# epsilla-cloud/vectordb

Measured on AMD Instinct MI355X. Metric: QPS @ recall@10>=0.999, 10Mx768 L2, higher is better.
Workload: dtype f32 (exact fp32 distances; the batched scan runs an int8 MFMA pass (int32 accumulation) over an 8-bit mirror of the rows as a lower-bound filter, survivors re-ranked in fp32)

## Files before the change

### vectordb_amd/build.py

```python
import os
import subprocess
import sys
from concurrent.futures import ThreadPoolExecutor

HERE = os.path.dirname(os.path.abspath(__file__))
SRC = os.path.join(HERE, "csrc")
OUT = os.path.join(HERE, "lib")
OBJ = os.path.join(OUT, "obj")
LIB = os.path.join(OUT, "libepsilla_gfx950.so")
SOURCES = ["index.cpp", "index_calls.cpp", "c_abi.cpp", "shard_group.cpp", "exchange.cpp", "flat_kernels.hip", "traverse.hip", "mfma_filter.hip", "one_pass.hip",
           "mirror_build.hip", "graph_build.hip", "select.hip", "range.hip"]
FLAGS = ["--offload-arch=gfx950", "-O3", "-std=c++17", "-fPIC", "-fno-gpu-rdc", "-Wall", "-Wno-unused-function",
         "-I" + os.path.join(os.path.dirname(HERE), "include")]


def _hipcc():
    for c in (os.environ.get("HIPCC"), "/opt/rocm/bin/hipcc", "hipcc"):
        if c and (os.path.sep not in c or os.path.exists(c)):
            return c
    raise RuntimeError("hipcc not found")


def _stale(target, deps):
    if not os.path.exists(target):
        return True
    t = os.path.getmtime(target)
    return any(os.path.getmtime(d) > t for d in deps)


def build(force=False, verbose=False):
    os.makedirs(OBJ, exist_ok=True)
    hipcc = _hipcc()
    headers = [os.path.join(SRC, f) for f in os.listdir(SRC) if f.endswith((".hpp", ".h"))]
    headers.append(os.path.join(os.path.dirname(HERE), "include", "epsilla_gfx950.h"))
    jobs = []
    objs = []
    for s in SOURCES:
        src = os.path.join(SRC, s)
        obj = os.path.join(OBJ, s.rsplit(".", 1)[0] + ".o")
        objs.append(obj)
        if force or _stale(obj, [src] + headers):
            cmd = [hipcc] + FLAGS + (["-x", "hip"] if s.endswith(".cpp") else []) + ["-c", src, "-o", obj]
            jobs.append(cmd)
# ... 21 lines not shown
```

### vectordb_amd/csrc/flat_kernels.hip

```cpp
#include "kernels.hpp"
#include "stream8_kernel.hpp"

namespace eps {

template <int NQ, int KPL>
__device__ __forceinline__ void offer(WaveTopK<KPL> (&list)[NQ], u64 (&thr)[NQ], int q, u64 key, bool valid,
                                      const FilterSpec& f, int k, bool unique) {
  u64 m = __ballot(valid && key < thr[q]);
  while (m) {
    const int l = __ffsll((long long)m) - 1;
    m &= m - 1;
    const u64 x = shfl64(key, l);
    if (x < thr[q] && row_visible(f, key_id(x), key_dist(x))) {
      if (unique) list[q].insert_unique(x); else list[q].insert(x);
      const u64 kth = list[q].entry(k - 1);
      thr[q] = kth < thr[q] ? kth : thr[q];
    }
  }
}

template <int NQ, int KPL, bool VEC4, int U>
__global__ __launch_bounds__(256) void flat_scan_kernel(FlatScanArgs a) {
  extern __shared__ __attribute__((aligned(16))) float smem[];
  const int dim = a.dim;
// ... 72 lines not shown
  if (gx_cap < 1) gx_cap = 1;
  int64_t gx = gx_rows < gx_cap ? gx_rows : gx_cap;
  return (int)(gx * 4);
}

template <int NQ, int KPL>
static void launch_flat_scan_t(const FlatScanArgs& a, bool vec4, hipStream_t s) {
  const int gx = a.W / 4;
  const int64_t groups = (a.nq + NQ - 1) / NQ;
  dim3 grid(gx, (unsigned)groups);
  const size_t shm = (size_t)NQ * ((a.dim + 3) & ~3) * sizeof(float);
  if (vec4)
    hipLaunchKernelGGL((flat_scan_kernel<NQ, KPL, true, 4>), grid, dim3(256), shm, s, a);
  else
    hipLaunchKernelGGL((flat_scan_kernel<NQ, KPL, false, 4>), grid, dim3(256), shm, s, a);
}

void launch_flat_scan(const FlatScanArgs& a, hipStream_t s) {
  if (a.nq <= 0 || a.row_end <= a.row_begin) return;
  const bool vec4 = (a.dim % 4 == 0) && ((reinterpret_cast<uintptr_t>(a.rows) & 15) == 0);
  const int kpl = pick_kpl(a.k);
  const int nq = pick_nq(a.nq, a.k, a.dim);
#define EPS_CASE(NQ_, KPL_) \
  if (nq == NQ_ && kpl == KPL_) return launch_flat_scan_t<NQ_, KPL_>(a, vec4, s);
  EPS_CASE(1, 1) EPS_CASE(2, 1) EPS_CASE(4, 1)
  EPS_CASE(1, 2) EPS_CASE(2, 2) EPS_CASE(4, 2)
  EPS_CASE(1, 4) EPS_CASE(1, 8) EPS_CASE(1, 16)
#undef EPS_CASE
}

template <int KPL, int NW>
__global__ __launch_bounds__(NW * 64) void merge_lists_kernel(const u64* partial, int lists, int k, u64* run_keys,
                                                          int merge_run, const u32* counts, FilterSpec vis, u64 id_stride, u32 id_head,
                                                          u32* seed_cand, int seed_cap, u32* seed_cnt) {
  __shared__ u64 sh[NW][KPL * 64];
  constexpr int NT = NW * 64;
  const int64_t q = blockIdx.x;
  const int lane = lane_id();
  const int wave = threadIdx.x >> 6;
  const u64* src = partial + q * (int64_t)lists;
  int total = lists;
  if (counts) total = counts[q] < (u32)total ? (int)counts[q] : total;
  WaveTopK<KPL> L[1];
  u64 thr[1];
  L[0].init();
  thr[0] = KEY_EMPTY;
  FilterSpec nof = {nullptr, nullptr, 0, 0, 0, 0};
  if (merge_run) {
    thr[0] = run_keys[q * k + (k - 1)];
    if (wave == 0) L[0].load(run_keys + q * k, k);
  }
  const int rounded = (total + NT - 1) / NT * NT;
  for (int i = threadIdx.x; i < rounded; i += NT) {
    const u64 key = i < total ? src[i] : KEY_EMPTY;
    if (id_stride) {
      const bool ok = key != KEY_EMPTY && row_visible(vis, seed_row(key_id(key), id_head, id_stride), key_dist(key));
      offer<1, KPL>(L, thr, 0, key, ok, nof, k, false);
    } else {
      offer<1, KPL>(L, thr, 0, key, key != KEY_EMPTY, vis, k, false);
    }
  }
  L[0].store(&sh[wave][0], k);
  __syncthreads();
  if (wave == 0) {
    for (int w = 1; w < NW; ++w) {
      for (int e0 = 0; e0 < k; e0 += 64) {
        const int e = e0 + lane;
        const u64 key = e < k ? sh[w][e] : KEY_EMPTY;
        offer<1, KPL>(L, thr, 0, key, key != KEY_EMPTY, nof, k, false);
      }
    }
    if (seed_cand) {
      int c = 0;
#pragma unroll
      for (int r = 0; r < KPL; ++r) {
        const int e = r * 64 + lane;
        const u64 key = L[0].key[r];
        const bool ok = e < k && key != KEY_EMPTY;
        const unsigned long long m = __ballot(ok);
        if (ok) seed_cand[q * (int64_t)seed_cap + c + __popcll(m & ((1ull << lane) - 1ull))] = id_stride ? seed_row(key_id(key), id_head, id_stride) : key_id(key);
        c += __popcll(m);
        if (e < k) run_keys[q * k + e] = KEY_EMPTY;
      }
      if (lane == 0) seed_cnt[q] = (u32)c;
    } else {
      L[0].store(run_keys + q * k, k);
    }
  }
}

void launch_merge_lists(const u64* partial, int lists, int k, int64_t nq, u64* run_keys, bool merge_run, hipStream_t s,
                        const u32* counts, const FilterSpec* visible, u64 id_stride, u32 id_head, u32* seed_cand, int seed_cap, u32* seed_cnt) {
  const FilterSpec vis = visible ? *visible : no_filter();
  if (nq <= 0) return;
  const int kpl = pick_kpl(k);
  const bool wide = nq <= 64 && kpl <= 2;
#define EPS_CASE(KPL_) \
  if (kpl == KPL_) {   \
    if (wide && KPL_ <= 2)                                                                                                                                       \
      hipLaunchKernelGGL((merge_lists_kernel<(KPL_ <= 2 ? KPL_ : 1), 16>), dim3((unsigned)nq), dim3(1024), 0, s, partial, lists, k, run_keys, merge_run ? 1 : 0, counts, vis, \
                         id_stride, id_head, seed_cand, seed_cap, seed_cnt);                                                                                      \
    else                                                                                                                                                         \
      hipLaunchKernelGGL((merge_lists_kernel<KPL_, 4>), dim3((unsigned)nq), dim3(256), 0, s, partial, lists, k, run_keys, merge_run ? 1 : 0, counts, vis, id_stride, id_head, \
                         seed_cand, seed_cap, seed_cnt);                                                                                                          \
    return;            \
  }
  EPS_CASE(1) EPS_CASE(2) EPS_CASE(4) EPS_CASE(8) EPS_CASE(16)
#undef EPS_CASE
}

template <int KPL, bool VEC4, int NW>
__global__ __launch_bounds__(NW * 64) void rerank_kernel(RerankArgs a) {
  extern __shared__ __attribute__((aligned(16))) float smem[];
  constexpr int NT = NW * 64;
  const int dim = a.dim;
  const int qstride = (dim + 3) & ~3;
  u64* sh = reinterpret_cast<u64*>(smem + qstride);
  const int64_t q = blockIdx.x;
  for (int i = threadIdx.x; i < qstride; i += NT) smem[i] = i < dim ? a.queries[q * dim + i] : 0.f;
  if (a.fuse && a.gsync && q == 0)
    for (int i = threadIdx.x; i < 256; i += NT) a.gsync[i] = 0;
  __syncthreads();
  const int lane = lane_id();
  const int wave = threadIdx.x >> 6;
  const int G = group_lanes(dim, VEC4);
  const int RPW = 64 / G;
  const int g = lane / G;
  const int t = lane & (G - 1);
  constexpr int U = 4;
  __shared__ u32 s8_kept, s8_lost;
  __shared__ int s8_T;
  if (a.s8_G) {
    if (threadIdx.x == 0) s8_kept = s8_lost = 0;
    if (wave == 0) {
      int gk;
      const int T = stream8_threshold_of(a.s8_G + q * (a.s8_slots * S8_SLOT_STRIDE), a.k, a.qstat + q * 4, a.scal, a.metric, a.u, a.slack, lane, gk, a.s8_slots);
      if (lane == 0) s8_T = T;
// ... 382 lines not shown
```

### vectordb_amd/csrc/kernels.hpp

```cpp
#pragma once
#include <hip/hip_runtime.h>
#include <stdint.h>

#include "device_common.hpp"

namespace eps {

struct FlatScanArgs {
  const float* rows;
  int64_t row_begin, row_end;
  int dim;
  int metric;
  const float* queries;
  int64_t nq;
  int k;
  FilterSpec f;
  u64* partial;
  int W;
  const u64* thr_in;
  const u64* lo_in;
  int64_t lo_stride;
};
int flat_scan_waves(int64_t nrows, int64_t nq, int dim);
void launch_flat_scan(const FlatScanArgs& a, hipStream_t s);

void launch_merge_lists(const u64* keys, int slots, int k, int64_t nq, u64* run_keys, bool merge_run, hipStream_t s,
                        const u32* counts = nullptr, const FilterSpec* visible = nullptr, u64 id_stride = 0, u32 id_head = 0,
                        u32* seed_cand = nullptr, int seed_cap = 0, u32* seed_cnt = nullptr);

struct RerankArgs {
  const float* rows;
  int dim;
  int metric;
  const float* queries;
  int64_t nq;
  int k;
  FilterSpec f;
  const u32* cand;
  u32* cand_count;
  int cap;
  u64* run_keys;
  int fuse;
  u32* overflow;
  unsigned long long* total;
  void* T_next;
  const float* qstat;
  const float* scal;
  int bits;
  float u, slack;
  u32* gsync;
  int64_t* fin_ids = nullptr;
  float* fin_dist = nullptr;
  int32_t* fin_counts = nullptr;
  int64_t fin_base = 0, fin_stride = 1;
  const int* s8_G = nullptr;
  int s8_slots = 64;
  const u32* s8_counts = nullptr;
  const u64* s8_lists = nullptr;
  int s8_waves = 0;
  u32* s8_cand = nullptr;
  u32* pub = nullptr;
// ... 82 lines not shown
```

### vectordb_amd/csrc/mfma_filter.hip

```cpp
#include <algorithm>
#include <cmath>
#include <cstdio>
#include <cstring>
#include <numeric>
#include <vector>

#include "mirror.hpp"
#include "mfma_kernels.hpp"

namespace eps {

__global__ __launch_bounds__(256) void query_prep_kernel(const float* q, int64_t nq, int64_t b_pad, int dim, int d_pad,
                                                         _Float16* qh, float* qstat) {
  const int64_t r = (int64_t)blockIdx.x * 4 + (threadIdx.x >> 6);
  if (r >= b_pad) return;
  const int lane = lane_id();
  _Float16* dst = qh + r * d_pad;
  if (r >= nq) {
    for (int c = lane; c < d_pad; c += 64) dst[c] = (_Float16)0.f;
    if (lane == 0) qstat[r * 4 + 0] = qstat[r * 4 + 1] = qstat[r * 4 + 2] = qstat[r * 4 + 3] = 0.f;
    return;
  }
  const float* src = q + r * dim;
  float s2 = 0.f, e2 = 0.f;
// ... 114 lines not shown
    bounds.push_back(approx ? S0 : 0);
    int nstages = i8 ? (nq <= 4 ? 3 : (nq <= 64 ? 4 : 6)) : 3;
    if (i8)
      while (nstages < 8 && (double)k * 5.0 * std::pow((double)n / (double)S0, 1.0 / (double)nstages) > 0.5 * (double)cap) ++nstages;
    const double r = std::max(i8 ? 3.0 : 4.0, std::pow((double)n / (double)S0, 1.0 / (double)nstages));
    const int64_t qt = std::max<int64_t>(1, b_pad / 256);
    const int64_t unit = 256 * std::max<int64_t>(1, 256 / std::gcd<int64_t>(256, qt));
    double f = 1.0;
    for (int st = 1; st < nstages; ++st) {
      f *= r;
      int64_t bnd = (int64_t)((double)S0 * f) / ROWPAD * ROWPAD;
      if (bnd >= 2 * unit) bnd = bnd / unit * unit;
      if (bnd < n && bnd > bounds.back()) bounds.push_back(bnd);
    }
  } else {
    bounds.push_back(std::min(S0, n));
    for (int64_t bnd : {S0 * 32, S0 * 256}) {
      if (bnd < n && bnd > bounds.back()) bounds.push_back(bnd);
    }
  }
  if (bounds.back() < n) bounds.push_back(n);
  return bounds;
}

struct Chain {
  const float* dq; int64_t nq; int k; u64* run_keys;
  bool i8;
  bool approx;
  int64_t n;
  bool fold;
  bool seeded;
  bool prologue;
  bool gsync;
  int version;
  int64_t b_pad, S0;
  int cap;
  int d_pad_h;
  float u8, slack;
  CallCounters c;
  FilterSpec fs;
  std::vector<int64_t> bounds;
  bool prep_does_it_all() const { return i8 && version >= 7; }
  const float* maxima(const HalfMirror& m) const { return i8 ? (fold ? m.scal8f.as<float>() : m.scal8.as<float>()) : m.scal.as<float>(); }
  u32* group_counters(const HalfMirror& m) const { return gsync ? m.gsync.as<u32>() : nullptr; }
};

static int32_t plan_chain(Index& ix, HalfMirror& m, const float* dq, int64_t nq, int k, u64* run_keys, bool approx, int cap_scale, bool i8, int64_t n, Chain* out) {
  Chain& c = *out = Chain{dq, nq, k, run_keys, i8, approx, n};
  c.b_pad = (nq + BN3 - 1) / BN3 * BN3;
  c.cap = std::max(4096, 64 * k) * cap_scale;
  c.d_pad_h = i8 ? m.d_pad8 / 2 : m.d_pad;
  c.u8 = key_unit8(ix.metric_, m.step8);
  c.slack = rerank_slack(ix.dim_);
  const int64_t b_pad = c.b_pad;
  if (!m.qstat.reserve((size_t)b_pad * 16) || !m.T.reserve((size_t)b_pad * 4) || !m.cand.reserve((size_t)nq * c.cap * 8) ||
      !m.cnt.reserve((size_t)(nq + 4) * 4 + 16) || !m.seedc.reserve((size_t)nq * k * 4) || !(i8 ? m.q8.reserve((size_t)b_pad * m.d_pad8) : m.qh.reserve((size_t)b_pad * m.d_pad * 2)))
    return ix.fail(EPS_INFRA_UNEXPECTED_ERROR, "MFMA engine: out of device memory (scratch)");
  c.version = (c.d_pad_h % 128 != 0 || c.d_pad_h < 256) ? 3 : 7;
  if (c.version >= 7 && !m.qf.reserve((size_t)b_pad * c.d_pad_h * 2)) return ix.fail(EPS_INFRA_UNEXPECTED_ERROR, "MFMA engine: out of device memory (scratch)");
  if (!m.gsync.reserve(1024)) return ix.fail(EPS_INFRA_UNEXPECTED_ERROR, "MFMA engine: out of device memory (scratch)");
  c.S0 = seed_rows(k);
  c.seeded = !(tune_int("EPS_MFMA_SEED", 1) == 0) && n > 4 * c.S0;
  c.prologue = c.seeded && c.version >= 7;
  c.gsync = !(tune_int("EPS_MFMA_GROUPSYNC", 1) == 0);
  c.fold = i8 && !approx && m.fold8;
  c.c = call_counters(m.cnt.as<u32>(), nq);
  c.fs = ix.filter_spec();
  c.bounds = plan_stages(n, nq, k, b_pad, c.cap, i8, approx, c.seeded);
  return EPS_OK;
}

static int32_t prepare_queries(Index& ix, HalfMirror& m, const Chain& c) {
  hipStream_t s = ix.stream_;
  if (c.i8) {
    Prep8Extra px;
    if (c.prep_does_it_all()) {
      px.qf = m.qf.as<signed char>();
      if (c.prologue) {
        px.T2 = reinterpret_cast<u64*>(m.T.p);
        px.n2 = c.b_pad / 2;
        px.Tv = 0x7F8000007F800000ull;
        px.cnt = c.c.cnt;
        px.cntv = (u32)c.S0;
        px.gsync = c.group_counters(m);
      }
    }
    const hipError_t er = prep8_queries(m, c.fold, (int)ix.dim_, ix.metric_, c.dq, c.nq, c.b_pad, m.q8.as<signed char>(), m.qstat.as<float>(), px, s);
    if (er != hipSuccess) return ix.hip_fail(er, "memset");
    if (c.fold) ix.stats_.i8_folded = 1;
    ix.stats_.i8_rotated = m.rot8 ? 1 : 0;
  } else {
    hipLaunchKernelGGL(query_prep_kernel, dim3((unsigned)((c.b_pad + 3) / 4)), dim3(256), 0, s, c.dq, c.nq, c.b_pad, (int)ix.dim_,
                       m.d_pad, m.qh.as<_Float16>(), m.qstat.as<float>());
  }
  if (c.version >= 7 && !c.prep_does_it_all())
    hipLaunchKernelGGL(pack_qf_kernel, dim3((unsigned)((c.b_pad / 32) * (c.d_pad_h / 16))), dim3(64), 0, s, m.qh.as<_Float16>(), m.qf.as<_Float16>(), c.b_pad, c.d_pad_h);
  return EPS_OK;
}

static FilterArgs filter_args(const Index& ix, const HalfMirror& m, const Chain& c) {
  const bool i8 = c.i8;
  FilterArgs fa;
  fa.xh = i8 ? reinterpret_cast<const _Float16*>(m.x8.p) : m.xh.as<_Float16>();
  fa.qh = i8 ? reinterpret_cast<const _Float16*>(m.q8.p) : m.qh.as<_Float16>();
  fa.qf = m.qf.as<_Float16>();
  fa.base = i8 ? (c.fold ? m.acc0b.as<float>() : m.acc0.as<float>()) : (ix.metric_ == 0 ? m.xn.as<float>() : m.zeros.as<float>());
  fa.base_s = i8 ? (c.fold ? m.acc0b.as<float>() : m.acc0.as<float>()) : (ix.metric_ == 0 ? m.xn_s.as<float>() : m.zeros_s.as<float>());
  fa.T = m.T.as<float>();
  fa.d_pad = c.d_pad_h;
  fa.tiles_q = (int)(c.b_pad / BN3);
  fa.nq = c.nq;
  fa.s = i8 ? -c.u8 : (ix.metric_ == 0 ? -2.f : -1.f);
  fa.inv_s = 1.f / fa.s;
  fa.cand = m.cand.as<u32>();
  fa.cand_keys = c.approx ? m.cand.as<u64>() : nullptr;
  fa.qstat = m.qstat.as<float>();
  fa.metric = ix.metric_;
  fa.cnt = c.c.cnt;
  fa.cap = c.cap;
  fa.group_sync = nullptr;
  fa.sync_shift = std::min(8, std::max(0, tune_int("EPS_MFMA_SYNC_SHIFT", 2)));
  fa.dense = 0;
  return fa;
}

constexpr size_t V3_LDS_BYTES = 2 * 65536 + 2 * 256 * sizeof(float);

static void ensure_filter_kernels(const Index& ix, HalfMirror& m) {
  if (m.num_cus) return;
  hipDeviceProp_t prop;
  m.num_cus = hipGetDeviceProperties(&prop, ix.device_) == hipSuccess ? prop.multiProcessorCount : 256;
  m.num_cus = m.num_cus / 8 * 8;
  if (m.num_cus < 8) m.num_cus = 8;
  (void)hipFuncSetAttribute(reinterpret_cast<const void*>(mfma_filter_kernel_v3), hipFuncAttributeMaxDynamicSharedMemorySize, (int)V3_LDS_BYTES);
  for (const void* fn : {reinterpret_cast<const void*>(mfma_filter_kernel_v7<2, FM_IDS>), reinterpret_cast<const void*>(mfma_filter_kernel_v7<2, FM_KEYS>),
                         reinterpret_cast<const void*>(mfma_filter_kernel_v7<2, FM_DENSE>), reinterpret_cast<const void*>(mfma_filter_kernel_v7<1, FM_IDS>),
                         reinterpret_cast<const void*>(mfma_filter_kernel_v7<1, FM_KEYS>), reinterpret_cast<const void*>(mfma_filter_kernel_v7<1, FM_DENSE>),
                         reinterpret_cast<const void*>(mfma_filter_kernel_v7<2, FM_IDS, true>), reinterpret_cast<const void*>(mfma_filter_kernel_v7<2, FM_KEYS, true>),
                         reinterpret_cast<const void*>(mfma_filter_kernel_v7<2, FM_DENSE, true>), reinterpret_cast<const void*>(mfma_filter_kernel_v7<1, FM_IDS, true>),
                         reinterpret_cast<const void*>(mfma_filter_kernel_v7<1, FM_KEYS, true>), reinterpret_cast<const void*>(mfma_filter_kernel_v7<1, FM_DENSE, true>)})
    (void)hipFuncSetAttribute(fn, hipFuncAttributeMaxDynamicSharedMemorySize, (int)V7_LDS_BYTES);
}

template <int JQ, bool I8>
static void launch_v7(const FilterArgs& f, dim3 grid, hipStream_t s) {
  const dim3 block(256);
  if (f.dense) hipLaunchKernelGGL((mfma_filter_kernel_v7<JQ, FM_DENSE, I8>), grid, block, V7_LDS_BYTES, s, f);
  else if (f.cand_keys) hipLaunchKernelGGL((mfma_filter_kernel_v7<JQ, FM_KEYS, I8>), grid, block, V7_LDS_BYTES, s, f);
  else hipLaunchKernelGGL((mfma_filter_kernel_v7<JQ, FM_IDS, I8>), grid, block, V7_LDS_BYTES, s, f);
}

static void launch_filter(const HalfMirror& m, const Chain& c, FilterArgs f, hipStream_t s) {
  const dim3 grid((unsigned)m.num_cus);
  if (c.version < 7) {
    hipLaunchKernelGGL(mfma_filter_kernel_v3, grid, dim3(512), V3_LDS_BYTES, s, f);
    return;
  }
  f.group_sync = c.group_counters(m);
  if (f.group_sync && f.dense && !c.prologue) (void)hipMemsetAsync(f.group_sync, 0, 1024, s);
  if (c.nq <= 128) {
    f.tiles_q = 1;
    if (c.i8) launch_v7<1, true>(f, grid, s); else launch_v7<1, false>(f, grid, s);
  } else {
    if (c.i8) launch_v7<2, true>(f, grid, s); else launch_v7<2, false>(f, grid, s);
  }
}

static int32_t run_seed_pass(Index& ix, HalfMirror& m, const Chain& c, const FilterArgs& fa, RerankArgs ra) {
  hipStream_t s = ix.stream_;
  const bool i8 = c.i8;
  const int64_t S0 = c.S0;
  u32* cnt = c.c.cnt;
  const bool dense = c.version >= 7;
  if (c.prologue && c.prep_does_it_all()) {
  } else if (c.prologue) {
    const int64_t cells = std::max<int64_t>(std::max<int64_t>(c.b_pad / 2, c.nq), 256);
    hipLaunchKernelGGL(seed_prologue_kernel, dim3((unsigned)((cells + 255) / 256)), dim3(256), 0, s, reinterpret_cast<u64*>(m.T.p), c.b_pad / 2, 0x7F8000007F800000ull,
                       cnt, c.nq, (u32)S0, c.group_counters(m));
  } else {
    launch_fill_u64(reinterpret_cast<u64*>(m.T.p), c.b_pad / 2, 0x7F8000007F800000ull, s);
    const hipError_t er = dense ? hipMemsetD32Async(reinterpret_cast<hipDeviceptr_t>(cnt), (int)S0, (size_t)c.nq, s) : hipMemsetAsync(cnt, 0, (size_t)c.nq * 4, s);
    if (er != hipSuccess) return ix.hip_fail(er, "memset");
  }
  unsigned long long seed_stride = 0;
  u32 seed_head = 0;
  FilterArgs f0 = fa;
  f0.dense = dense ? 1 : 0;
  f0.cand_keys = m.cand.as<u64>();
  if (!c.approx) {
    const u32 sample_head = (u32)(S0 / 2);
    const unsigned long long sample_stride = (unsigned long long)(((unsigned __int128)(c.n - sample_head) << 32) / (unsigned __int128)(S0 - sample_head));
    int64_t& smp_version = i8 ? m.sample8_version : m.sample_version;
    int64_t& smp_n = i8 ? m.sample8_n : m.sample_n;
    int64_t& smp_rows = i8 ? m.sample8_rows : m.sample_rows;
    DevBuf& smp_x = i8 ? m.sx8 : m.sxh;
    DevBuf& smp_base = i8 ? m.sacc0 : m.sbase;
    DevBuf& smp_base_u = i8 ? m.sacc0 : m.sbase_u;
    if (smp_version != ix.rows_version_ || smp_n != c.n || smp_rows != S0) {
      if (!smp_x.reserve((size_t)S0 * c.d_pad_h * 2) || !smp_base.reserve((size_t)S0 * 4) || !smp_base_u.reserve((size_t)S0 * 4))
        return ix.fail(EPS_INFRA_UNEXPECTED_ERROR, "MFMA engine: out of device memory (seed sample)");
      hipLaunchKernelGGL(seed_sample_kernel, dim3((unsigned)S0), dim3(256), 0, s, fa.xh, i8 ? m.acc0.as<u32>() : reinterpret_cast<const u32*>(fa.base_s),
                         i8 ? m.acc0.as<u32>() : reinterpret_cast<const u32*>(fa.base),
                         sample_stride, sample_head, c.d_pad_h, smp_x.as<_Float16>(), smp_base.as<u32>(), smp_base_u.as<u32>());
      smp_version = ix.rows_version_;
      smp_n = c.n;
      smp_rows = S0;
    }
    f0.xh = smp_x.as<_Float16>();
    f0.base_s = smp_base.as<float>();
    f0.base = smp_base_u.as<float>();
    seed_stride = sample_stride;
    seed_head = sample_head;
  }
  f0.tile0 = 0;
  f0.ntiles = (S0 + BM3 - 1) / BM3;
  f0.row_hi = S0;
  launch_filter(m, c, f0, s);
  if (c.approx) {
    launch_merge_lists(f0.cand_keys, c.cap, c.k, c.nq, c.run_keys, false, s, cnt, nullptr, seed_stride, seed_head);
    return EPS_OK;
  }
  launch_merge_lists(f0.cand_keys, c.cap, c.k, c.nq, c.run_keys, false, s, cnt, &c.fs, seed_stride, seed_head, m.seedc.as<u32>(), c.k, cnt);
  ra.cand = m.seedc.as<u32>();
  ra.cap = c.k;
  ra.fuse = 2;
  ra.T_next = m.T.p;
  launch_rerank(ra, s);
  return EPS_OK;
}

static void dump_stage(const HalfMirror& m, const Chain& c, size_t st, int64_t ntiles, hipStream_t s) {
  const int64_t nq = c.nq;
  const int k = c.k;
  std::vector<u32> hc((size_t)nq);
  std::vector<float> hT((size_t)nq);
  std::vector<u64> hk((size_t)nq * k);
  (void)hipMemcpyAsync(hc.data(), c.c.cnt, (size_t)nq * 4, hipMemcpyDeviceToHost, s);
  (void)hipMemcpyAsync(hT.data(), m.T.p, (size_t)nq * 4, hipMemcpyDeviceToHost, s);
  (void)hipMemcpyAsync(hk.data(), c.run_keys, (size_t)nq * k * 8, hipMemcpyDeviceToHost, s);
  (void)hipStreamSynchronize(s);
  u32 mn = ~0u, mx = 0; double sum = 0; float tmin = 3e38f, tmax = -3e38f; int64_t empt = 0, big = 0;
  for (int64_t j = 0; j < nq; ++j) { mn = std::min(mn, hc[j]); mx = std::max(mx, hc[j]); sum += hc[j]; tmin = std::min(tmin, hT[j]); tmax = std::max(tmax, hT[j]); empt += hk[j * k + k - 1] == KEY_EMPTY; big += hc[j] > (u32)c.cap; }
  fprintf(stderr, "[eps] stage %zu rows [%lld,%lld) tiles %lld: cnt min %u mean %.1f max %u (>cap: %lld), T min %g max %g, empty kth %lld, scal %g %g %g\n", st, (long long)c.bounds[st], (long long)c.bounds[st + 1], (long long)ntiles, mn, sum / nq, mx, (long long)big, tmin, tmax, (long long)empt, m.h_scal[0], m.h_scal[1], m.h_scal[2]);
}

static void run_stage(Index& ix, HalfMirror& m, const Chain& c, size_t st, FilterArgs fa, RerankArgs ra, bool* fin_done) {
  hipStream_t s = ix.stream_;
  const int64_t lo = c.bounds[st], hi = c.bounds[st + 1];
  const bool fused = !c.approx;
  const bool have_T = fused && (st > 0 || c.seeded);
  const int pad_only = have_T ? 1 : 0;
  if ((!have_T || st == 0) && !(have_T && c.i8 && c.prologue)) {
    const dim3 grid((unsigned)((c.b_pad + 255) / 256));
    if (c.i8)
      hipLaunchKernelGGL(threshold8_kernel, grid, dim3(256), 0, s, c.run_keys, c.k, c.nq, c.b_pad, m.qstat.as<float>(), c.maxima(m), ix.metric_, c.u8, m.T.as<int>(), c.c.cnt,
// ... 399 lines not shown
```

### vectordb_amd/csrc/mfma_kernels.hpp

```cpp
#pragma once
#include <hip/hip_runtime.h>
#include <stdint.h>

#include <type_traits>

#include "device_common.hpp"

namespace eps {

typedef _Float16 half8 __attribute__((ext_vector_type(8)));
typedef float f32x16 __attribute__((ext_vector_type(16)));
typedef int i32x16 __attribute__((ext_vector_type(16)));


struct FilterArgs {
  const _Float16* xh;
  const _Float16* qh;
  const _Float16* qf;
  const float* base;
  const float* base_s;
  int dense;
  u32* group_sync;
  int sync_shift;
  const float* T;
// ... 48 lines not shown
template <bool I8> struct V7Op;
template <> struct V7Op<false> {
  typedef half8 frag;
  typedef f32x16 accv;
  typedef float scalar;
  static __device__ __forceinline__ scalar max16(const accv& v) { return max16f(v); }
};
template <> struct V7Op<true> {
  typedef i32x4 frag;
  typedef i32x16 accv;
  typedef int scalar;
  static __device__ __forceinline__ scalar max16(const accv& v) { return max16i(v); }
};

constexpr int V7_VI = 7;
#define EPS_FRAG_C "=a"
template <bool I8> struct V7Asm;
template <> struct V7Asm<true> {
  template <class A, class F> static __device__ __forceinline__ void v(A& acc, const F& a, const F& b) { asm volatile("v_mfma_i32_32x32x32_i8 %0, %1, %2, %0" : "+v"(acc) : "a"(a), "a"(b)); }
  template <class A, class F> static __device__ __forceinline__ void a_(A& acc, const F& a, const F& b) { asm volatile("v_mfma_i32_32x32x32_i8 %0, %1, %2, %0" : "+a"(acc) : "a"(a), "a"(b)); }
  template <class A, class F> static __device__ __forceinline__ void v2(A& d, const F& a, const F& b, const A& c) { asm volatile("v_mfma_i32_32x32x32_i8 %0, %1, %2, %3" : "=&v"(d) : "a"(a), "a"(b), "v"(c)); }
  template <class A, class F> static __device__ __forceinline__ void a2(A& d, const F& a, const F& b, const A& c) { asm volatile("v_mfma_i32_32x32x32_i8 %0, %1, %2, %3" : "=&a"(d) : "a"(a), "a"(b), "a"(c)); }
};
template <> struct V7Asm<false> {
  template <class A, class F> static __device__ __forceinline__ void v(A& acc, const F& a, const F& b) { asm volatile("v_mfma_f32_32x32x16_f16 %0, %1, %2, %0" : "+v"(acc) : "a"(a), "a"(b)); }
  template <class A, class F> static __device__ __forceinline__ void a_(A& acc, const F& a, const F& b) { asm volatile("v_mfma_f32_32x32x16_f16 %0, %1, %2, %0" : "+a"(acc) : "a"(a), "a"(b)); }
  template <class A, class F> static __device__ __forceinline__ void v2(A& d, const F& a, const F& b, const A& c) { asm volatile("v_mfma_f32_32x32x16_f16 %0, %1, %2, %3" : "=&v"(d) : "a"(a), "a"(b), "v"(c)); }
  template <class A, class F> static __device__ __forceinline__ void a2(A& d, const F& a, const F& b, const A& c) { asm volatile("v_mfma_f32_32x32x16_f16 %0, %1, %2, %3" : "=&a"(d) : "a"(a), "a"(b), "a"(c)); }
};

__device__ __forceinline__ int swz(int row, int chunk) { return (row << 3) + (chunk ^ ((row >> 1) & 7)); }

constexpr int BM3 = 256, BN3 = 256;
__global__ __launch_bounds__(512, 2) void mfma_filter_kernel_v3(FilterArgs a) {
  extern __shared__ __attribute__((aligned(16))) unsigned char lds[];
  constexpr int SLOT = 65536;
  const int tid = threadIdx.x;
  const int lane = tid & 63;
  const int wave = tid >> 6;
  const int wm = wave >> 2, wn = wave & 3;
  const int khalf = lane >> 5;
  float* base_lds = reinterpret_cast<float*>(lds + 2 * SLOT);

  const int xcd = blockIdx.x & 7;
  const int local = blockIdx.x >> 3;
  const int per_xcd = gridDim.x >> 3;
  const int QTB = a.tiles_q < per_xcd ? a.tiles_q : per_xcd;
  const int G = per_xcd / QTB;
  const int qslot = local % QTB;
  const int rg = local / QTB;
  if (rg >= G) return;
  const int64_t nj = (a.ntiles - xcd + 7) / 8;
  const int nqt = (a.tiles_q - qslot + QTB - 1) / QTB;
  const int64_t my_rows = nj > rg ? (nj - rg + G - 1) / G : 0;
  const int64_t ntile = my_rows * nqt;
  if (ntile <= 0) return;
  const int ldk = a.d_pad;
  const int KT = ldk / BK;

  int g_off[4];
#pragma unroll
  for (int it = 0; it < 4; ++it) {
    const int s = it * 512 + tid;
    const int row = s >> 3;
    g_off[it] = row * ldk + ((s & 7) ^ ((row >> 1) & 7)) * 8;
  }
// ... 115 lines not shown
    }
#pragma unroll
    for (int i = 0; i < 4; ++i) {
      const int rbase = wm * 128 + i * 32 + 4 * khalf;
#pragma unroll
      for (int j = 0; j < 2; ++j) {
        float mx = acc[i][j][0];
#pragma unroll
        for (int r = 1; r < 16; ++r) mx = fmaxf(mx, acc[i][j][r]);
        if (__any(mx >= Tq[j])) {
#pragma unroll
          for (int r = 0; r < 16; ++r) {
            if (acc[i][j][r] >= Tq[j]) {
              const int64_t row = row0 + rbase + (r & 3) + 8 * (r >> 2);
              if (row < a.row_hi && qj[j] < a.nq) {
                const u32 slot_c = atomicAdd(&a.cnt[qj[j]], 1u);
                if (slot_c < (u32)a.cap) {
                  if (a.cand_keys) {
                    float dapx = acc[i][j][r] * a.s + cj[j];
                    if (a.metric == 0) dapx = fmaxf(dapx, 0.f);
                    a.cand_keys[qj[j] * (int64_t)a.cap + slot_c] = make_key(dapx, (u32)row);
                  } else {
                    a.cand[qj[j] * (int64_t)a.cap + slot_c] = (u32)row;
                  }
                }
              }
            }
          }
        }
      }
    }
  }
}

#define EPS_DS_READ_B128(dst, addr, off) asm volatile("ds_read_b128 %0, %1 offset:%2" : EPS_FRAG_C(dst) : "v"(addr), "n"(off))
#define EPS_GLOAD_B128(dst, voff, sbase, off) \
  asm volatile("global_load_dwordx4 %0, %1, %2 offset:%3" : EPS_FRAG_C(dst) : "v"(voff), "s"(sbase), "n"(off))

enum { FM_IDS = 0, FM_KEYS = 1, FM_DENSE = 2 };
constexpr int V7_CAPW = 128;
constexpr size_t V7_LDS_BYTES = (size_t)4 * 256 * 128 + 2 * 256 * sizeof(float) + 4096 + 64 + 4 * V7_CAPW * (8 + 4);

template <int JQ, int MODE, bool I8 = false>
__global__ __launch_bounds__(256, 1) void mfma_filter_kernel_v7(FilterArgs a) {
  constexpr int NRB = 8;
  constexpr int TR = 32 * NRB;
  constexpr int VI = V7_VI;
  constexpr int GROUP = 2;
  typedef V7Op<I8> OP;
  typedef typename OP::frag frag_t;
  typedef typename OP::accv acc_t;
  typedef typename OP::scalar thr_t;
  constexpr int QT = 128 * JQ;
  extern __shared__ __attribute__((aligned(16))) unsigned char lds[];
  constexpr int ASLOT = TR * 128;
  constexpr int RING = 4;
  const int tid = threadIdx.x;
  const int lane = tid & 63;
  const int wave = __builtin_amdgcn_readfirstlane(tid >> 6);
  const int l31 = lane & 31;
  float* base_lds = reinterpret_cast<float*>(lds + RING * ASLOT);

  const int xcd = blockIdx.x & 7;
  const int local = blockIdx.x >> 3;
  const int per_xcd = gridDim.x >> 3;
  const int QTB = a.tiles_q < per_xcd ? a.tiles_q : per_xcd;
  const int G = per_xcd / QTB;
  const int qslot = local % QTB;
  const int rg = local / QTB;
  if (rg >= G) return;
  const int64_t nj = (a.ntiles - xcd + 7) / 8;
  const int nqt = (a.tiles_q - qslot + QTB - 1) / QTB;
  const int64_t my_rows = nj > rg ? (nj - rg + G - 1) / G : 0;
  const int64_t ntile = my_rows * nqt;
  if (ntile <= 0) return;
  const int ldk = a.d_pad;
  const int KT = ldk / 64;
// ... 35 lines not shown
  int64_t qj[JQ];
  float* tq_lds = base_lds + 512 + wave * 256;
#pragma unroll
  for (int j = 0; j < JQ; ++j) {
    qj[j] = (int64_t)qslot * QT + wave * (32 * JQ) + j * 32 + l31;
    tq_lds[j * 64 + lane] = I8 ? a.T[qj[j]] : a.T[qj[j]] * a.inv_s;
    tq_lds[(2 + j) * 64 + lane] = MODE != FM_IDS ? (I8 ? a.qstat[qj[j] * 4 + 3] : (a.metric == 0 ? a.qstat[qj[j] * 4] : (a.metric == 1 ? 1.f : 0.f))) : 0.f;
  }
  u32 faddr[4];
  auto lane_values = [&]() __attribute__((always_inline)) {
    u32 ln;
    asm volatile("v_mbcnt_lo_u32_b32 %0, -1, 0\n\tv_mbcnt_hi_u32_b32 %0, -1, %0" : "=v"(ln));
    lane16 = ln * 16;
    lane4 = ln * 4;
    const u32 td = (u32)wave * 64 + ln, row = td >> 3;
    g_off0 = (row * (u32)ldk + ((td & 7) ^ ((row >> 1) & 7)) * 8) * 2;
#pragma unroll
    for (int kk = 0; kk < 4; ++kk) faddr[kk] = lds_base + (u32)swz((int)(ln & 31), kk * 2 + (int)(ln >> 5)) * 16;
  };
  lane_values();

  const int64_t a_stride = (int64_t)8 * G * TR * ldk;
  int ri_c = 0, qi_c = 0;
  int ri_n = 0, qi_n = 0;
  advance(ri_n, qi_n);
  const _Float16* A_t = rows_of(0);
  const _Float16* A_n = ntile > 1 ? rows_of(ri_n) : A_t;
  const _Float16* B_t = frags_of(0);
  const _Float16* B_n = (nqt > 1 && ntile > 1) ? frags_of(qi_n) : B_t;
  u32* wcnt = reinterpret_cast<u32*>(lds + RING * ASLOT + 2048 + 4096) + wave * 4;
  u64* wbuf = reinterpret_cast<u64*>(lds + RING * ASLOT + 2048 + 4096 + 64) + wave * V7_CAPW;
  float* wkey = reinterpret_cast<float*>(lds + RING * ASLOT + 2048 + 4096 + 64 + 4 * V7_CAPW * 8) + wave * V7_CAPW;
  volatile __attribute__((address_space(3))) u32* wcnt_lds = (volatile __attribute__((address_space(3))) u32*)wcnt;
  if (MODE != FM_DENSE && lane == 0) *wcnt = 0;
  auto append = [&](int64_t qq, u32 row, float dapx) __attribute__((always_inline)) {
    const u32 slot_c = atomicAdd(&a.cnt[qq], 1u);
    if (slot_c < (u32)a.cap) {
      if (MODE == FM_KEYS) a.cand_keys[qq * (int64_t)a.cap + slot_c] = make_key(dapx, row);
      else a.cand[qq * (int64_t)a.cap + slot_c] = row;
    }
  };
  auto flush = [&]() __attribute__((always_inline)) {
    u32 ln;
    asm volatile("v_mbcnt_lo_u32_b32 %0, -1, 0\n\tv_mbcnt_hi_u32_b32 %0, -1, %0" : "=v"(ln));
    u32 n = *wcnt_lds;
    n = n < (u32)V7_CAPW ? n : (u32)V7_CAPW;
    for (u32 e = ln; e < n; e += 64) {
      const u64 v = wbuf[e];
      append((int64_t)(v >> 32), (u32)v, MODE == FM_KEYS ? wkey[e] : 0.f);
    }
    if (ln == 0) *wcnt_lds = 0;
  };
  const bool rendezvous = a.group_sync && a.tiles_q <= per_xcd;
  u32* gs_ctr = a.group_sync + (xcd * G + rg);
  const int64_t sync_mask = ((int64_t)1 << a.sync_shift) - 1;
  if (rendezvous && wave == 0 && lane == 0) __hip_atomic_fetch_add(gs_ctr, 1u, __ATOMIC_RELAXED, __HIP_MEMORY_SCOPE_AGENT);
  asm volatile("s_waitcnt vmcnt(0)" ::: "memory");
  issue_base(0, 0);
#pragma unroll
  for (int it = 0; it < NRB; ++it) issue_piece(A_t, 0, it);
#pragma unroll
  for (int it = 0; it < NRB; ++it) issue_piece(A_t + 64, ASLOT, it);
#pragma unroll
  for (int kk = 0; kk < 4; ++kk) {
    EPS_GLOAD_B128(fb[0][kk][0], lane16, B_t + kk * 512, 0);
    if (JQ == 2) EPS_GLOAD_B128(fb[0][kk][JQ - 1], lane16, B_t + jstride + kk * 512, 0);
  }
// ... 177 lines not shown
  }
      EPS_INIT_AT_HEAD(0) EPS_INIT_AT_HEAD(1) EPS_INIT_AT_HEAD(2) EPS_INIT_AT_HEAD(3)
      EPS_INIT_AT_HEAD(4) EPS_INIT_AT_HEAD(5) EPS_INIT_AT_HEAD(6) EPS_INIT_AT_HEAD(7)
#undef EPS_INIT_AT_HEAD
    }
    step(std::integral_constant<int, 0>{}, std::true_type{});
    step(std::integral_constant<int, 1>{}, std::false_type{});
    for (int kt = 2; kt < KT; kt += 2) {
      step(std::integral_constant<int, 0>{}, std::false_type{});
      step(std::integral_constant<int, 1>{}, std::false_type{});
    }
    asm volatile("s_nop 15\n\ts_nop 7" ::: "memory");
    if (rendezvous && wave == 0 && t + 1 < ntile && ((t + 1) & sync_mask) == 0 && lane16 == 0) __hip_atomic_fetch_add(gs_ctr, 1u, __ATOMIC_RELAXED, __HIP_MEMORY_SCOPE_AGENT);
    A_t = A_n;
    B_t = B_n;
    ri_c = ri_n;
    qi_c = qi_n;
    {
      const int ri_before = ri_n;
      advance(ri_n, qi_n);
      if (t + 2 < ntile) {
        if (ri_n != ri_before) A_n += a_stride;
        if (nqt > 1) B_n = frags_of(qi_n);
      }
    }
    u32 lne;
    asm volatile("v_mbcnt_lo_u32_b32 %0, -1, 0\n\tv_mbcnt_hi_u32_b32 %0, -1, %0" : "=v"(lne));
    const int l31e = (int)(lne & 31), kh4e = (int)(lne >> 5) * 4;
    thr_t Tq[JQ];
    float cj[JQ];
#pragma unroll
    for (int j = 0; j < JQ; ++j) {
      Tq[j] = __builtin_bit_cast(thr_t, tq_lds[j * 64 + lne]);
      cj[j] = MODE == FM_DENSE ? tq_lds[(2 + j) * 64 + lne] : 0.f;
    }
#pragma unroll
    for (int i0 = 0; i0 < NRB; i0 += GROUP) {
      thr_t mxg[GROUP][JQ];
      bool group_hit = true;
      if (MODE != FM_DENSE) {
        bool h = false;
#pragma unroll
        for (int j = 0; j < JQ; ++j) {
          __builtin_amdgcn_sched_barrier(0);
          thr_t gm = mxg[0][j] = OP::max16(acc[i0][j]);
#pragma unroll
          for (int ii = 1; ii < GROUP; ++ii) {
            __builtin_amdgcn_sched_barrier(0);
            mxg[ii][j] = OP::max16(acc[i0 + ii][j]);
            gm = gm > mxg[ii][j] ? gm : mxg[ii][j];
          }
          h |= gm >= Tq[j];
        }
        group_hit = __any(h);
      }
      if (MODE == FM_DENSE || __builtin_expect(group_hit, 0)) {
#pragma unroll
        for (int ii = 0; ii < GROUP; ++ii) {
          const int i = i0 + ii;
          const int rbase = i * 32 + kh4e;
#pragma unroll
          for (int j = 0; j < JQ; ++j) {
            __builtin_amdgcn_sched_barrier(0);
            if (MODE == FM_DENSE) {
              const int64_t qq = qbase + j * 32 + l31e;
              if (qq < a.nq) {
#pragma unroll
                for (int r = 0; r < 16; ++r) {
                  const int64_t row = row0 + rbase + (r & 3) + 8 * (r >> 2);
                  float dapx = (float)acc[i][j][r] * a.s + cj[j];
                  const bool nan = dapx != dapx;
                  if (a.metric == 0) dapx = fmaxf(dapx, 0.f);
                  if (row < a.row_hi)
                    a.cand_keys[qq * (int64_t)a.cap + (row - a.tile0 * TR)] =
                        nan ? KEY_EMPTY : make_key(dapx, (u32)row);
                }
              }
              continue;
            }
            if (__any(mxg[ii][j] >= Tq[j])) {
              int l31h = l31e, rbh = rbase;
              asm volatile("" : "+v"(l31h), "+v"(rbh));
              const int64_t qq = qbase + j * 32 + l31h;
              u32 hm = 0;
#pragma unroll
              for (int r = 0; r < 16; ++r) hm |= acc[i][j][r] >= Tq[j] ? (1u << r) : 0u;
              if (qq >= a.nq) hm = 0;
              while (hm) {
                const int r = __builtin_ctz(hm);
                hm &= hm - 1;
                const int64_t row64 = row0 + rbh + (r & 3) + 8 * (r >> 2);
                if (row64 >= a.row_hi) continue;
                const u32 row = (u32)row64;
                float dapx = 0.f;
                if (MODE == FM_KEYS) {
                  thr_t v = acc[i][j][0];
#pragma unroll
                  for (int rr = 1; rr < 16; ++rr) v = r == rr ? acc[i][j][rr] : v;
                  dapx = (float)v * a.s + tq_lds[(2 + j) * 64 + lne];
                  if (a.metric == 0) dapx = fmaxf(dapx, 0.f);
                }
                const u32 e = atomicAdd(wcnt, 1u);
                if (e < (u32)V7_CAPW) {
                  wbuf[e] = ((u64)qq << 32) | row;
                  if (MODE == FM_KEYS) wkey[e] = dapx;
                } else {
                  append(qq, row, dapx);
                }
              }
            }
          }
        }
      }
    }
    if (MODE != FM_DENSE) {
      if (*wcnt_lds >= (u32)(V7_CAPW / 2)) flush();
    }
  }
  if (MODE != FM_DENSE) flush();
  asm volatile("s_waitcnt vmcnt(0)" ::: "memory");
}


__global__ void pack_qf_kernel(const _Float16* qh, _Float16* qf, int64_t b_pad, int d_pad) {
  const int64_t frag = blockIdx.x;
  const int KC = d_pad / 16;
  const int64_t qb = frag / KC;
  const int kc = (int)(frag % KC);
  const int lane = threadIdx.x;
  const half8 v = *reinterpret_cast<const half8*>(qh + (qb * 32 + (lane & 31)) * d_pad + kc * 16 + (lane >> 5) * 8);
  *reinterpret_cast<half8*>(qf + (frag * 64 + lane) * 8) = v;
}


}
```

Measured before the change: 140,400.

## Seed pass keeps only best row per 16-row block, transposed layout

Adds an FM_SEED mode to the v7 MFMA filter kernel. For each 16-row group it emits only the best approximate key, so the seed stage writes S0/16 slots per query instead of S0. The output is stored query-minor and read by the merge kernel through a new element stride. This shrinks the seed candidate writes and the merge work, at the risk of a looser initial threshold because only the per-block best rows survive. The mode is used only for unfiltered exact v7 runs and can be turned off with EPS_MFMA_SEED=2.

```diff
diff --git a/vectordb_amd/build.py b/vectordb_amd/build.py
--- a/vectordb_amd/build.py
+++ b/vectordb_amd/build.py
@@ -8,7 +8,7 @@
 OUT = os.path.join(HERE, "lib")
 OBJ = os.path.join(OUT, "obj")
 LIB = os.path.join(OUT, "libepsilla_gfx950.so")
-SOURCES = ["index.cpp", "index_calls.cpp", "c_abi.cpp", "shard_group.cpp", "exchange.cpp", "flat_kernels.hip", "traverse.hip", "mfma_filter.hip", "one_pass.hip",
+SOURCES = ["index.cpp", "index_calls.cpp", "c_abi.cpp", "shard_group.cpp", "exchange.cpp", "flat_kernels.hip", "traverse.hip", "mfma_filter.hip", "seed_pass.hip", "one_pass.hip",
            "mirror_build.hip", "graph_build.hip", "select.hip", "range.hip"]
 FLAGS = ["--offload-arch=gfx950", "-O3", "-std=c++17", "-fPIC", "-fno-gpu-rdc", "-Wall", "-Wno-unused-function",
          "-I" + os.path.join(os.path.dirname(HERE), "include")]
diff --git a/vectordb_amd/csrc/flat_kernels.hip b/vectordb_amd/csrc/flat_kernels.hip
--- a/vectordb_amd/csrc/flat_kernels.hip
+++ b/vectordb_amd/csrc/flat_kernels.hip
@@ -128,13 +128,14 @@
 template <int KPL, int NW>
 __global__ __launch_bounds__(NW * 64) void merge_lists_kernel(const u64* partial, int lists, int k, u64* run_keys,
                                                           int merge_run, const u32* counts, FilterSpec vis, u64 id_stride, u32 id_head,
-                                                          u32* seed_cand, int seed_cap, u32* seed_cnt) {
+                                                          u32* seed_cand, int seed_cap, u32* seed_cnt, int64_t e_stride) {
   __shared__ u64 sh[NW][KPL * 64];
   constexpr int NT = NW * 64;
   const int64_t q = blockIdx.x;
   const int lane = lane_id();
   const int wave = threadIdx.x >> 6;
-  const u64* src = partial + q * (int64_t)lists;
+  const u64* src = e_stride ? partial + q : partial + q * (int64_t)lists;
+  const int64_t es = e_stride ? e_stride : 1;
   int total = lists;
   if (counts) total = counts[q] < (u32)total ? (int)counts[q] : total;
   WaveTopK<KPL> L[1];
@@ -148,7 +149,7 @@
   }
   const int rounded = (total + NT - 1) / NT * NT;
   for (int i = threadIdx.x; i < rounded; i += NT) {
-    const u64 key = i < total ? src[i] : KEY_EMPTY;
+    const u64 key = i < total ? src[i * es] : KEY_EMPTY;
     if (id_stride) {
       const bool ok = key != KEY_EMPTY && row_visible(vis, seed_row(key_id(key), id_head, id_stride), key_dist(key));
       offer<1, KPL>(L, thr, 0, key, ok, nof, k, false);
@@ -186,7 +187,7 @@
 }
 
 void launch_merge_lists(const u64* partial, int lists, int k, int64_t nq, u64* run_keys, bool merge_run, hipStream_t s,
-                        const u32* counts, const FilterSpec* visible, u64 id_stride, u32 id_head, u32* seed_cand, int seed_cap, u32* seed_cnt) {
+                        const u32* counts, const FilterSpec* visible, u64 id_stride, u32 id_head, u32* seed_cand, int seed_cap, u32* seed_cnt, int64_t e_stride) {
   const FilterSpec vis = visible ? *visible : no_filter();
   if (nq <= 0) return;
   const int kpl = pick_kpl(k);
@@ -195,10 +196,10 @@
   if (kpl == KPL_) {   \
     if (wide && KPL_ <= 2)                                                                                                                                       \
       hipLaunchKernelGGL((merge_lists_kernel<(KPL_ <= 2 ? KPL_ : 1), 16>), dim3((unsigned)nq), dim3(1024), 0, s, partial, lists, k, run_keys, merge_run ? 1 : 0, counts, vis, \
-                         id_stride, id_head, seed_cand, seed_cap, seed_cnt);                                                                                      \
+                         id_stride, id_head, seed_cand, seed_cap, seed_cnt, e_stride);                                                                            \
     else                                                                                                                                                         \
       hipLaunchKernelGGL((merge_lists_kernel<KPL_, 4>), dim3((unsigned)nq), dim3(256), 0, s, partial, lists, k, run_keys, merge_run ? 1 : 0, counts, vis, id_stride, id_head, \
-                         seed_cand, seed_cap, seed_cnt);                                                                                                          \
+                         seed_cand, seed_cap, seed_cnt, e_stride);                                                                                                \
     return;            \
   }
   EPS_CASE(1) EPS_CASE(2) EPS_CASE(4) EPS_CASE(8) EPS_CASE(16)
diff --git a/vectordb_amd/csrc/kernels.hpp b/vectordb_amd/csrc/kernels.hpp
--- a/vectordb_amd/csrc/kernels.hpp
+++ b/vectordb_amd/csrc/kernels.hpp
@@ -26,7 +26,7 @@
 
 void launch_merge_lists(const u64* keys, int slots, int k, int64_t nq, u64* run_keys, bool merge_run, hipStream_t s,
                         const u32* counts = nullptr, const FilterSpec* visible = nullptr, u64 id_stride = 0, u32 id_head = 0,
-                        u32* seed_cand = nullptr, int seed_cap = 0, u32* seed_cnt = nullptr);
+                        u32* seed_cand = nullptr, int seed_cap = 0, u32* seed_cnt = nullptr, int64_t e_stride = 0);
 
 struct RerankArgs {
   const float* rows;
diff --git a/vectordb_amd/csrc/mfma_filter.hip b/vectordb_amd/csrc/mfma_filter.hip
--- a/vectordb_amd/csrc/mfma_filter.hip
+++ b/vectordb_amd/csrc/mfma_filter.hip
@@ -170,6 +170,8 @@
   bool seeded;
   bool prologue;
   bool gsync;
+  bool seed_best;
+  int seed_slots;
   int version;
   int64_t b_pad, S0;
   int cap;
@@ -201,9 +203,12 @@
   c.seeded = !(tune_int("EPS_MFMA_SEED", 1) == 0) && n > 4 * c.S0;
   c.prologue = c.seeded && c.version >= 7;
   c.gsync = !(tune_int("EPS_MFMA_GROUPSYNC", 1) == 0);
+  const bool seed_v7 = c.seeded && !approx && c.version >= 7;
+  c.fs = ix.filter_spec();
+  c.seed_best = seed_v7 && !(c.fs.deleted || c.fs.column || c.fs.prog) && tune_int("EPS_MFMA_SEED", 1) != 2;
+  c.seed_slots = (int)(c.seed_best ? c.S0 / 16 : c.S0);
   c.fold = i8 && !approx && m.fold8;
   c.c = call_counters(m.cnt.as<u32>(), nq);
-  c.fs = ix.filter_spec();
   c.bounds = plan_stages(n, nq, k, b_pad, c.cap, i8, approx, c.seeded);
   return EPS_OK;
 }
@@ -219,7 +224,7 @@
         px.n2 = c.b_pad / 2;
         px.Tv = 0x7F8000007F800000ull;
         px.cnt = c.c.cnt;
-        px.cntv = (u32)c.S0;
+        px.cntv = (u32)c.seed_slots;
         px.gsync = c.group_counters(m);
       }
     }
@@ -278,6 +283,7 @@
                          reinterpret_cast<const void*>(mfma_filter_kernel_v7<2, FM_DENSE, true>), reinterpret_cast<const void*>(mfma_filter_kernel_v7<1, FM_IDS, true>),
                          reinterpret_cast<const void*>(mfma_filter_kernel_v7<1, FM_KEYS, true>), reinterpret_cast<const void*>(mfma_filter_kernel_v7<1, FM_DENSE, true>)})
     (void)hipFuncSetAttribute(fn, hipFuncAttributeMaxDynamicSharedMemorySize, (int)V7_LDS_BYTES);
+  seed_filter_kernels_init();
 }
 
 template <int JQ, bool I8>
@@ -296,8 +302,10 @@
   }
   f.group_sync = c.group_counters(m);
   if (f.group_sync && f.dense && !c.prologue) (void)hipMemsetAsync(f.group_sync, 0, 1024, s);
-  if (c.nq <= 128) {
-    f.tiles_q = 1;
+  if (c.nq <= 128) f.tiles_q = 1;
+  if (f.dense == 2) {
+    launch_seed_filter(f, grid.x, c.nq <= 128, c.i8, s);
+  } else if (c.nq <= 128) {
     if (c.i8) launch_v7<1, true>(f, grid, s); else launch_v7<1, false>(f, grid, s);
   } else {
     if (c.i8) launch_v7<2, true>(f, grid, s); else launch_v7<2, false>(f, grid, s);
@@ -314,16 +322,16 @@
   } else if (c.prologue) {
     const int64_t cells = std::max<int64_t>(std::max<int64_t>(c.b_pad / 2, c.nq), 256);
     hipLaunchKernelGGL(seed_prologue_kernel, dim3((unsigned)((cells + 255) / 256)), dim3(256), 0, s, reinterpret_cast<u64*>(m.T.p), c.b_pad / 2, 0x7F8000007F800000ull,
-                       cnt, c.nq, (u32)S0, c.group_counters(m));
+                       cnt, c.nq, (u32)c.seed_slots, c.group_counters(m));
   } else {
     launch_fill_u64(reinterpret_cast<u64*>(m.T.p), c.b_pad / 2, 0x7F8000007F800000ull, s);
-    const hipError_t er = dense ? hipMemsetD32Async(reinterpret_cast<hipDeviceptr_t>(cnt), (int)S0, (size_t)c.nq, s) : hipMemsetAsync(cnt, 0, (size_t)c.nq * 4, s);
+    const hipError_t er = dense ? hipMemsetD32Async(reinterpret_cast<hipDeviceptr_t>(cnt), c.seed_slots, (size_t)c.nq, s) : hipMemsetAsync(cnt, 0, (size_t)c.nq * 4, s);
     if (er != hipSuccess) return ix.hip_fail(er, "memset");
   }
   unsigned long long seed_stride = 0;
   u32 seed_head = 0;
   FilterArgs f0 = fa;
-  f0.dense = dense ? 1 : 0;
+  f0.dense = c.seed_best ? 2 : (dense ? 1 : 0);
   f0.cand_keys = m.cand.as<u64>();
   if (!c.approx) {
     const u32 sample_head = (u32)(S0 / 2);
@@ -358,7 +366,7 @@
     launch_merge_lists(f0.cand_keys, c.cap, c.k, c.nq, c.run_keys, false, s, cnt, nullptr, seed_stride, seed_head);
     return EPS_OK;
   }
-  launch_merge_lists(f0.cand_keys, c.cap, c.k, c.nq, c.run_keys, false, s, cnt, &c.fs, seed_stride, seed_head, m.seedc.as<u32>(), c.k, cnt);
+  launch_merge_lists(f0.cand_keys, c.cap, c.k, c.nq, c.run_keys, false, s, cnt, &c.fs, seed_stride, seed_head, m.seedc.as<u32>(), c.k, cnt, c.seed_best ? c.nq : 0);
   ra.cand = m.seedc.as<u32>();
   ra.cap = c.k;
   ra.fuse = 2;
diff --git a/vectordb_amd/csrc/mfma_kernels.hpp b/vectordb_amd/csrc/mfma_kernels.hpp
--- a/vectordb_amd/csrc/mfma_kernels.hpp
+++ b/vectordb_amd/csrc/mfma_kernels.hpp
@@ -104,6 +104,7 @@
 __device__ __forceinline__ int swz(int row, int chunk) { return (row << 3) + (chunk ^ ((row >> 1) & 7)); }
 
 constexpr int BM3 = 256, BN3 = 256;
+#ifndef EPS_MFMA_V7_TEMPLATE_ONLY
 __global__ __launch_bounds__(512, 2) void mfma_filter_kernel_v3(FilterArgs a) {
   extern __shared__ __attribute__((aligned(16))) unsigned char lds[];
   constexpr int SLOT = 65536;
@@ -285,17 +286,19 @@
     }
   }
 }
+#endif
 
 #define EPS_DS_READ_B128(dst, addr, off) asm volatile("ds_read_b128 %0, %1 offset:%2" : EPS_FRAG_C(dst) : "v"(addr), "n"(off))
 #define EPS_GLOAD_B128(dst, voff, sbase, off) \
   asm volatile("global_load_dwordx4 %0, %1, %2 offset:%3" : EPS_FRAG_C(dst) : "v"(voff), "s"(sbase), "n"(off))
 
-enum { FM_IDS = 0, FM_KEYS = 1, FM_DENSE = 2 };
+enum { FM_IDS = 0, FM_KEYS = 1, FM_DENSE = 2, FM_SEED = 3 };
 constexpr int V7_CAPW = 128;
 constexpr size_t V7_LDS_BYTES = (size_t)4 * 256 * 128 + 2 * 256 * sizeof(float) + 4096 + 64 + 4 * V7_CAPW * (8 + 4);
 
 template <int JQ, int MODE, bool I8 = false>
 __global__ __launch_bounds__(256, 1) void mfma_filter_kernel_v7(FilterArgs a) {
+  constexpr bool LISTS = MODE == FM_IDS || MODE == FM_KEYS;
   constexpr int NRB = 8;
   constexpr int TR = 32 * NRB;
   constexpr int VI = V7_VI;
@@ -397,7 +400,7 @@
   u64* wbuf = reinterpret_cast<u64*>(lds + RING * ASLOT + 2048 + 4096 + 64) + wave * V7_CAPW;
   float* wkey = reinterpret_cast<float*>(lds + RING * ASLOT + 2048 + 4096 + 64 + 4 * V7_CAPW * 8) + wave * V7_CAPW;
   volatile __attribute__((address_space(3))) u32* wcnt_lds = (volatile __attribute__((address_space(3))) u32*)wcnt;
-  if (MODE != FM_DENSE && lane == 0) *wcnt = 0;
+  if (LISTS && lane == 0) *wcnt = 0;
   auto append = [&](int64_t qq, u32 row, float dapx) __attribute__((always_inline)) {
     const u32 slot_c = atomicAdd(&a.cnt[qq], 1u);
     if (slot_c < (u32)a.cap) {
@@ -641,13 +644,13 @@
 #pragma unroll
     for (int j = 0; j < JQ; ++j) {
       Tq[j] = __builtin_bit_cast(thr_t, tq_lds[j * 64 + lne]);
-      cj[j] = MODE == FM_DENSE ? tq_lds[(2 + j) * 64 + lne] : 0.f;
+      cj[j] = !LISTS ? tq_lds[(2 + j) * 64 + lne] : 0.f;
     }
 #pragma unroll
     for (int i0 = 0; i0 < NRB; i0 += GROUP) {
       thr_t mxg[GROUP][JQ];
       bool group_hit = true;
-      if (MODE != FM_DENSE) {
+      if (LISTS) {
         bool h = false;
 #pragma unroll
         for (int j = 0; j < JQ; ++j) {
@@ -663,7 +666,7 @@
         }
         group_hit = __any(h);
       }
-      if (MODE == FM_DENSE || __builtin_expect(group_hit, 0)) {
+      if (!LISTS || __builtin_expect(group_hit, 0)) {
 #pragma unroll
         for (int ii = 0; ii < GROUP; ++ii) {
           const int i = i0 + ii;
@@ -685,6 +688,24 @@
                         nan ? KEY_EMPTY : make_key(dapx, (u32)row);
                 }
               }
+              continue;
+            }
+            if (MODE == FM_SEED) {
+              const int64_t qq = qbase + j * 32 + l31e;
+              const int64_t blk = row0 + i * 32;
+              const thr_t mx = OP::max16(acc[i][j]);
+              u32 hm = 0;
+#pragma unroll
+              for (int r = 0; r < 16; ++r) hm |= acc[i][j][r] == mx ? (1u << r) : 0u;
+              u64 key = KEY_EMPTY;
+              if (hm && blk < a.row_hi) {
+                const int r = __builtin_ctz(hm);
+                float dapx = (float)mx * a.s + cj[j];
+                const bool nan = dapx != dapx;
+                if (a.metric == 0) dapx = fmaxf(dapx, 0.f);
+                if (!nan) key = make_key(dapx, (u32)(blk + kh4e + (r & 3) + 8 * (r >> 2)));
+              }
+              if (qq < a.nq) a.cand_keys[((blk - a.tile0 * TR) / 16 + (kh4e >> 2)) * a.nq + qq] = key;
               continue;
             }
             if (__any(mxg[ii][j] >= Tq[j])) {
@@ -722,15 +743,19 @@
         }
       }
     }
-    if (MODE != FM_DENSE) {
+    if (LISTS) {
       if (*wcnt_lds >= (u32)(V7_CAPW / 2)) flush();
     }
   }
-  if (MODE != FM_DENSE) flush();
+  if (LISTS) flush();
   asm volatile("s_waitcnt vmcnt(0)" ::: "memory");
 }
 
-
+void seed_filter_kernels_init();
+void launch_seed_filter(const FilterArgs& f, unsigned grid, bool one_tile, bool i8, hipStream_t s);
+
+
+#ifndef EPS_MFMA_V7_TEMPLATE_ONLY
 __global__ void pack_qf_kernel(const _Float16* qh, _Float16* qf, int64_t b_pad, int d_pad) {
   const int64_t frag = blockIdx.x;
   const int KC = d_pad / 16;
@@ -740,6 +765,7 @@
   const half8 v = *reinterpret_cast<const half8*>(qh + (qb * 32 + (lane & 31)) * d_pad + kc * 16 + (lane >> 5) * 8);
   *reinterpret_cast<half8*>(qf + (frag * 64 + lane) * 8) = v;
 }
+#endif
 
 
 }
diff --git a/vectordb_amd/csrc/seed_pass.hip b/vectordb_amd/csrc/seed_pass.hip
--- /dev/null
+++ b/vectordb_amd/csrc/seed_pass.hip
@@ -0,0 +1,23 @@
+#define EPS_MFMA_V7_TEMPLATE_ONLY
+#include "mfma_kernels.hpp"
+
+namespace eps {
+
+void seed_filter_kernels_init() {
+  for (const void* fn : {reinterpret_cast<const void*>(mfma_filter_kernel_v7<2, FM_SEED>), reinterpret_cast<const void*>(mfma_filter_kernel_v7<1, FM_SEED>),
+                         reinterpret_cast<const void*>(mfma_filter_kernel_v7<2, FM_SEED, true>), reinterpret_cast<const void*>(mfma_filter_kernel_v7<1, FM_SEED, true>)})
+    (void)hipFuncSetAttribute(fn, hipFuncAttributeMaxDynamicSharedMemorySize, (int)V7_LDS_BYTES);
+}
+
+void launch_seed_filter(const FilterArgs& f, unsigned grid, bool one_tile, bool i8, hipStream_t s) {
+  const dim3 g(grid), block(256);
+  if (one_tile) {
+    if (i8) hipLaunchKernelGGL((mfma_filter_kernel_v7<1, FM_SEED, true>), g, block, V7_LDS_BYTES, s, f);
+    else hipLaunchKernelGGL((mfma_filter_kernel_v7<1, FM_SEED, false>), g, block, V7_LDS_BYTES, s, f);
+  } else {
+    if (i8) hipLaunchKernelGGL((mfma_filter_kernel_v7<2, FM_SEED, true>), g, block, V7_LDS_BYTES, s, f);
+    else hipLaunchKernelGGL((mfma_filter_kernel_v7<2, FM_SEED, false>), g, block, V7_LDS_BYTES, s, f);
+  }
+}
+
+}
```

Result: no change. 141,100, median of 6 (+0.5%).
